# TimD1/vcfdist

Hardware: AMD Instinct MI355X
Metric: supercluster-alignments/sec (higher is better)
Workload: dtype int32; 1 GPU; wgs_synth; superclusters_per_gpu=1000000, span_dist=lognormal(median 20, sigma 1.2) clip [4,10000]

## Files before the change

### vcfdist_amd/csrc/pr_api.hip

```cpp
#include <hip/hip_runtime.h>
#include <hip/hip_ext.h>
#include <dlfcn.h>

#include <algorithm>
#include <atomic>
#include <chrono>
#include <cstdarg>
#include <cstdio>
#include <cstdlib>
#include <cstring>
#include <condition_variable>
#include <deque>
#include <functional>
#include <mutex>
#include <string>
#include <thread>
#include <tuple>
#include <unordered_map>
#include <unordered_set>
#include <vector>

#include "../../include/vcfdist_pr.h"
#include "pr_device.h"
#include "pr_plan.h"
// ... 910 lines not shown
    {
        static const int tie_model = vpr_selfcheck_tie_model(14);
        if (tie_model < 0)
            return fail(nullptr, VPR_ERR_STATE, "this machine's libstdc++ grows std::unordered_set through other bucket counts than the tie "
                        "replay's model (entry %d of TIE_BUCKET_LIST, pr_tie.hip): results on alignments with tied swap predecessors "
                        "would differ from a reference built here", -tie_model - 1);
    }
    int ndev = 0;
    hipError_t e = hipGetDeviceCount(&ndev);
    if (e != hipSuccess || ndev <= 0)
        return fail(nullptr, VPR_ERR_DEVICE, "no HIP device available (%s); this library has no CPU fallback",
                    e == hipSuccess ? "device count 0" : hipGetErrorString(e));
    if (cfg->device < 0 || cfg->device >= ndev)
        return fail(nullptr, VPR_ERR_ARG, "device %d out of range (have %d)", cfg->device, ndev);
    vpr_handle *h = new vpr_handle();
    h->cfg = *cfg;
    h->debug = getenv("VPR_DEBUG") != nullptr;
    h->no_strips = getenv("VPR_NO_STRIPS") != nullptr;
    h->no_round_overlap = getenv("VPR_NO_ROUND_OVERLAP") != nullptr;
    h->stall_log = getenv("VPR_STALL_LOG") != nullptr;
    h->seq_walk = getenv("VPR_SEQ_WALK") != nullptr;
    h->no_flag_save = getenv("VPR_NO_FLAG_SAVE") != nullptr;
    h->side_credit = exp_getenv("VPR_NO_SIDE_CREDIT") == nullptr;
    if (const char *e = exp_getenv("VPR_ZL_LDS_KB")) h->zl_lds_bytes = std::max(0, std::min(64, atoi(e))) * 1024;
    if (const char *e = exp_getenv("VPR_LANE_PRIO_ROWS")) h->lane_prio_rows = std::max(1, atoi(e));
    for (int k = 0; k < 2; k++)
        if (hipEventCreateWithFlags(&h->ev_cred[k], hipEventDisableTiming) != hipSuccess) return fail(nullptr, VPR_ERR_DEVICE, "hipEventCreate failed");
    if (const char *e = getenv("VPR_LONG_LT")) { const int v = atoi(e); if (v >= 64 && v <= 2048) h->long_lt = v; }
    memset(&h->dB, 0, sizeof(h->dB));
    memset(&h->timing, 0, sizeof(h->timing));
    const char *prio_map = exp_getenv("VPR_STREAM_PRIO");
    if (prio_map && strlen(prio_map) != size_t(N_CLASSES + 5)) prio_map = nullptr;
    if (hipSetDevice(cfg->device) != hipSuccess) { delete h; return fail(nullptr, VPR_ERR_DEVICE, "hipSetDevice failed"); }
    int prio_lo = 0, prio_hi = 0;
    (void)hipDeviceGetStreamPriorityRange(&prio_lo, &prio_hi);
    auto prio_of = [&](int idx, int dflt) { return !prio_map ? dflt : (prio_map[idx] == 'h' ? prio_hi : (prio_map[idx] == 'l' ? prio_lo : (prio_hi + prio_lo) / 2)); };
    if (hipStreamCreateWithPriority(&h->stream, exp_getenv("VPR_MAIN_BLOCKING") ? hipStreamDefault : hipStreamNonBlocking, prio_of(N_CLASSES + 4, (prio_hi + prio_lo) / 2)) != hipSuccess) {
        delete h;
        return fail(nullptr, VPR_ERR_DEVICE, "hipStreamCreate failed");
    }
    {
        size_t free_b = 0, total_b = 0;
        if (hipMemGetInfo(&free_b, &total_b) != hipSuccess) { delete h; return fail(nullptr, VPR_ERR_DEVICE, "hipMemGetInfo failed"); }
        h->dev_total = int64_t(total_b);
        h->tie_scratch_max = std::max<int64_t>(h->dev_total / 16, int64_t(64) << 20);
        h->lad_arena_max = std::max<int64_t>(h->dev_total / 8, int64_t(64) << 20);
// ... 1226 lines not shown
        });
        if (rc) return rc;
        }
        if (!(phases & 4)) return rc;
        const bool wave_walk = !q16 && (long_part || cnt < 2048);
        int64_t walk_rows_sum = 0;
        if (lv == LV_C1 && !h->seq_walk)
            for (int32_t k = 0; k < cnt && walk_rows_sum <= WSEG_MAX_ROWS; k++) walk_rows_sum += plan_desc(h, P, size_t(off) + size_t(k)).Lt;
        const bool seg_walk = lv == LV_C1 && !h->seq_walk && walk_rows_sum <= WSEG_MAX_ROWS;
        const bool row_walk = lv == LV_C1 && (wave_walk || seg_walk);
        vpr_launch_stat ws_;
        memset(&ws_, 0, sizeof(ws_));
        ws_.threads = q16 ? 16 : 64; ws_.n_units = cnt; ws_.cells_per_thread = 2;
        if (q16) {
            if (!zero) rc = timed(3, ws_, ks, "k_walk_q16", [&] {
                hipLaunchKernelGGL(k_walk_q16, dim3((cnt + 3) / 4), dim3(64), 0, ks, h->dB, h->d_descs, list, cnt,
                                   P.arena, a_i32, h->d_outs, a_path, tag, dtag, n_dev);
            });
            if (rc) return rc;
            ws_.cells_per_thread = 3;
            if (zero) {
                ws_.bytes_algorithmic = 20 * zl_rows;
                rc = timed(3, ws_, ks, "k_zero_walk", [&] {
                    hipLaunchKernelGGL(k_zero_walk, dim3((cnt + 63) / 64), dim3(64), 0, ks, h->d_descs, list, cnt, h->d_zl_hdr + zl_wave0,
                                       h->d_zl_in, h->d_zl_log, h->d_outs, a_path, (h->cfg.flags & VPR_CFG_KEEP_PATHS) ? 1 : 0, tag,
                                       h->lane_prio_rows);
                });
                if (rc) return rc;
                ws_.bytes_algorithmic = 0;
            }
            if (zero) rc = timed(3, ws_, ks, "k_zero_credit", [&] {
                hipLaunchKernelGGL(k_zero_credit, dim3((cnt + 63) / 64), dim3(64), 0, ks, h->dB, h->d_descs, list, cnt,
                                   h->d_zl_hdr + zl_wave0, h->d_zl_log, h->d_outs, h->d_secs, h->d_fp_table, h->d_jobs,
                                   h->d_njobs, h->jobs_cap, tag);
            });
            else if (cnt <= CREDIT_WAVE_MAX && !n_dev) rc = timed(3, ws_, ks, "k_credit<wave>", [&] {
                hipLaunchKernelGGL(k_credit<true>, dim3(cnt), dim3(64), 0, ks, h->dB, h->d_descs, list, cnt,
                                   h->d_outs, a_path, h->d_secs, h->d_fp_table, h->d_jobs, h->d_njobs,
                                   h->jobs_cap, dtag, tag, n_dev);
            });
            else {
                static const int head_max = [] { const char *e = exp_getenv("VPR_CREDIT_HEAD"); return e ? atoi(e) : 4096; }();
                const int32_t head = (n_dev && h->d_d1_blk && cnt > 2 * head_max) ? head_max : 0;
                if (head > 0) {
                    vpr_launch_stat wh_ = ws_;
                    wh_.n_units = head;
                    rc = timed(3, wh_, ks, "k_credit<wave>", [&] {
                        hipLaunchKernelGGL(k_credit<true>, dim3(head), dim3(64), 0, ks, h->dB, h->d_descs, list, head,
                                           h->d_outs, a_path, h->d_secs, h->d_fp_table, h->d_jobs, h->d_njobs,
                                           h->jobs_cap, dtag, tag, n_dev, 0);
                    });
                    if (rc) return rc;
                }
                rc = timed(3, ws_, ks, "k_credit<lane>", [&] {
                    hipLaunchKernelGGL(k_credit<false>, dim3((cnt - head + 63) / 64), dim3(64), 0, ks, h->dB, h->d_descs,
// ... 77 lines not shown
        const int nw = (cap + 63) / 64;
        vpr_launch_stat ls;
        memset(&ls, 0, sizeof(ls));
        ls.threads = 64; ls.cells_per_thread = 1; ls.n_units = cap;
        int rc = VPR_OK;
        if (ph == 1) {
            rc = timed(0, ls, ks, "k_prep_d1", [&] {
                hipLaunchKernelGGL(k_d1_hdr, dim3(nw), dim3(64), 0, ks, h->d_descs, list, n_dev, cap, h->d_outs, h->d_d1_hdr);
                hipLaunchKernelGGL(k_d1_scan, dim3(1), dim3(D1_SCAN_NT), 0, ks, h->d_d1_hdr, nw, h->d1_in_cap, h->d1_log_cap, h->d_d1_info);
                hipLaunchKernelGGL(k_prep_d1, dim3(nw), dim3(256), 0, ks, h->dB, h->d_descs, list, n_dev, cap, h->d_outs, h->d_d1_hdr, h->d_d1_in);
            });
            if (rc) return rc;
            rc = timed(1, ls, ks, "k_one_lane", [&] {
                hipLaunchKernelGGL(k_one_lane, dim3(nw), dim3(64), 0, ks, h->d_descs, list, n_dev, cap, h->d_d1_hdr, h->d_d1_in, h->d_d1_log,
                                   h->d_outs, reinterpret_cast<PathEnt *>(h->plan0.arena), (h->cfg.flags & VPR_CFG_KEEP_PATHS) ? 1 : 0, h->d_d1_info,
                                   std::max(1, h->lane_prio_rows / 4));
                hipLaunchKernelGGL(k_fwd_band_finish, dim3((cap + 255) / 256), dim3(256), 0, ks, list, cap, h->d_outs, D1_TAG, n_dev);
            });
            if (rc) return rc;
            ordered_fails(list, n_all, h->d_d1_fail, h->d_d1_info + 2, n_dev, ks);
        } else if (ph == 4) {
            ls.cells_per_thread = 3;
            rc = timed(3, ls, ks, "k_one_walk", [&] {
                hipLaunchKernelGGL(k_one_walk, dim3(nw), dim3(64), 0, ks, h->d_descs, list, n_dev, cap, h->d_d1_hdr, h->d_d1_in, h->d_d1_log,
                                   h->d_outs, reinterpret_cast<PathEnt *>(h->plan0.arena), (h->cfg.flags & VPR_CFG_KEEP_PATHS) ? 1 : 0, h->d_d1_info,
                                   std::max(1, h->lane_prio_rows / 4));
            });
            if (rc) return rc;
            rc = timed(3, ls, ks, "k_one_credit", [&] {
                hipLaunchKernelGGL(k_one_credit, dim3(nw), dim3(64), 0, ks, h->dB, h->d_descs, list, n_dev, cap, h->d_d1_hdr, h->d_d1_log,
                                   h->d_outs, h->d_secs, h->d_fp_table, h->d_jobs, h->d_njobs, h->jobs_cap, ztag);
            });
        }
        return rc;
    }

    int read_fails(int slot, int64_t fail_off, hipStream_t ls, std::vector<int32_t> &fails) {
        HIPCHK(h, x_event_sync(h, h->ev_slot[slot], SITE));
        const int32_t nf = h->hp_cnt[slot];
        if (nf > 0) {
            const size_t f0 = fails.size();
            fails.insert(fails.end(), h->hp_fail + fail_off, h->hp_fail + fail_off + nf);
            if (h->debug && nf <= (getenv("VPR_DEBUG_REJECTS") ? atoi(getenv("VPR_DEBUG_REJECTS")) : 64)) {
                for (size_t k = f0; k < fails.size(); k++) {
                    const int32_t a = fails[k];
                    AlnOut o;
                    (void)hipMemcpyAsync(&o, h->d_outs + a, sizeof(o), hipMemcpyDeviceToHost, ls);
                    (void)x_sync(h, ls, SITE);
                    const AlnDesc &d = h->descs[a];
                    fprintf(stderr, "[vpr] level %d rejected sc %d aln %d: Lq %d Lr %d Lt %d  s %d exit_min %d dq %d dr %d\n",
                            int(h->level[a]), d.sc, d.aln, d.Lq, d.Lr, d.Lt, o.s, o.exit_min, o.dist_q, o.dist_r);
                }
            }
// ... 910 lines not shown
```

### vcfdist_amd/csrc/pr_d1.hip

```cpp
#ifndef PR_D1_HIP_
#define PR_D1_HIP_

#define D1_TAG 9
#define D1_CLEAN ZL_CLEAN_REJECT

#define GE_ALIVE 1u
#define GE_MAT 2u
#define GE_SWP 4u
#define GE_PSLOT_SHIFT 3
#define GE_SUB 32u
#define GE_SUB_SHIFT 6
#define GE_INS 256u
#define GE_INS_SHIFT 9
#define GE_DEL 2048u
#define GE_DEL_SHIFT 12
#define GE_TP 16384u
#define GE_BWD 32768u

#define MV_SWP_R 0
#define MV_MAT 1
#define MV_SUB 2
#define MV_INS 3
#define MV_DEL 4
#define MV_SWP_Q 5
// ... 582 lines not shown
        zl_u4 pg_n = g_row(bmax - 1);
        for (int t = bmax - 1; t >= 0; t--) {
            const bool act = t < nrow;
            const bool first = act && t == nrow - 1;
            const zl_u2 pf = pf_n;
            const zl_u4 pgv = pg_n;
            pf_n = f_row(t - 1);
            pg_n = g_row(t - 1);
            const bool upper = act && ((((cf[0] | cf[1] | pf.x | pf.y) & 0xffff0000u) | cg[0][1] | cg[1][1] | pgv.y | pgv.w) != 0u);
#ifdef D1_CLOCKS
            if (lane == 0) { atomicAdd(info + 14, 1); if (__any(upper)) atomicAdd(info + 15, 1); }
#endif
            if (__any(upper)) sc_row(S4{}, t, act, first, pf, pgv);
            else sc_row(S2{}, t, act, first, pf, pgv);
        }
        beg_plane = kf[0][0] >= 0 ? VPR_PLANE_QUERY : VPR_PLANE_REF;
        ok = ok && (kf[0][0] >= 0 || kf[1][0] >= 0);
    }

    lapck(2);
    if (ok) { AlnOut &o = outs[a]; o.beg_plane = beg_plane; o.path_len = -1; }
}

__global__ void __launch_bounds__(64, 8) k_one_walk(const AlnDesc *__restrict__ descs, const int32_t *__restrict__ list,
                                                    const int32_t *__restrict__ n_dev, int n_cap, const ZlWave *__restrict__ hdr,
                                                    const uint32_t *__restrict__ zin, uint4 *__restrict__ zlog,
                                                    AlnOut *__restrict__ outs, PathEnt *__restrict__ paths, int keep_paths,
                                                    int32_t *__restrict__ info, int prio_rows) {
    const int w = blockIdx.x, lane = threadIdx.x;
    const ZlWave H = hdr[w];
    if (H.mt <= 0) return;
    if (H.mt >= prio_rows) __builtin_amdgcn_s_setprio(2);
    const int n_list = min(*n_dev, n_cap);
    const int wi = w * 64 + lane;
    const int a_ = wi < n_list ? list[wi] : -1;
    const int a = max(a_, 0);
    const AlnDesc *dp = descs + a;
    const bool ok = a_ >= 0 && outs[a].band_ok == D1_TAG && outs[a].path_len == -1;
    const int Lq = ok ? dp->Lq : 1, Lr = ok ? dp->Lr : 1;
    const int L[2] = {Lq, Lr};
    const int nrow = ok ? dp->Lt : 0;
    int bmax = nrow;
#pragma unroll
    for (int o = 32; o; o >>= 1) bmax = max(bmax, __shfl_xor(bmax, o));
    if (bmax == 0) return;
    const auto rin = __builtin_amdgcn_make_buffer_rsrc(const_cast<uint32_t *>(zin + H.in_off), 0, 256 * (2 * H.mq + 2 * H.mr + H.mt), 0x00020000);
    const auto rlog = __builtin_amdgcn_make_buffer_rsrc(zlog + H.log_off, 0, 2560 * (H.mt + 1), 0x00020000);
    const uint32_t lane4 = uint32_t(lane) << 2, lane8 = uint32_t(lane) << 3, lane16 = uint32_t(lane) << 4;
    const uint32_t posW[2] = {0u, uint32_t(2 * H.mq) << 8};
    const uint32_t post = uint32_t(2 * H.mq + 2 * H.mr) << 8;
    const uint32_t logB1 = uint32_t(H.mt + 1) << 10;
    auto in_at = [&](uint32_t off) -> uint32_t { return __builtin_amdgcn_raw_buffer_load_b32(rin, off, 0, 0); };
    auto word_at = [&](int p, int x, bool on) -> uint32_t { return in_at(on ? posW[p] + (uint32_t(x) << 8) + lane4 : ZL_OOB); };
    auto t_at = [&](int t, bool on) -> uint32_t { return in_at(on ? post + (uint32_t(t) << 8) + lane4 : ZL_OOB); };
    const int beg_plane = ok ? outs[a].beg_plane : 0;
    auto lapck = [&](int) {};
    {
        PathEnt *path = paths + dp->path_off;
        const uint32_t logS0 = logB1;
        int hi = beg_plane, slot = 0, layer = 0, x = 0, ti = 0, mv_in = -1;
        uint32_t status = 0;
        bool wok = ok, done = !ok;
        int plen = 0;
        for (int i = 0; i <= bmax; i++) {
            const bool act = wok && !done;
            if (!__any(act)) break;
            const uint32_t mvw = __builtin_amdgcn_raw_buffer_load_b32(rlog, act ? (uint32_t(ti) << 10) + lane16 + (uint32_t(layer) << 3) + (uint32_t(hi) << 2) : ZL_OOB, 0, 0);
            const uint32_t tw = t_at(ti, act);
            const uint32_t cw = word_at(hi, x, act);
            const int trv = ZW_PTR(tw), qref = hi ? x : ZW_PTR(cw);
            uint32_t sync = 1, edit = 0;
            if (mv_in >= 0) {
                const bool diag = mv_in != MV_INS && mv_in != MV_DEL;
                const bool in_t = (tw & ZW_PV) && !(tw & ZW_PB);
                const bool in_q = hi == 0 && (cw & ZW_PV) && !(cw & ZW_PB);
                sync = (diag && !in_t && !in_q && !((tw | cw) & ZW_INS) && trv == qref) ? 1u : 0u;
                edit = (mv_in == MV_SUB || mv_in == MV_INS || mv_in == MV_DEL) ? 1u : 0u;
            }
            const uint32_t eqb = (ZW_BASE(cw) == ZW_BASE(tw) ? 1u : 0u) | ((hi || !(cw & ZW_PV)) ? 2u : 0u);
            zl_u2 st;
            st.x = uint32_t(x) | (uint32_t(hi) << 16) | (sync << 17) | (eqb << 18) | (edit << 20) | (uint32_t(i - ti) << 21);
            st.y = uint32_t(qref + 1) | (uint32_t(trv + 1) << 16);
            __builtin_amdgcn_raw_buffer_store_b64(st, rlog, act ? logS0 + (uint32_t(i) << 9) + lane8 : ZL_OOB, 0, 0);
            if ((keep_paths & 1) && act) {
                uint4 pe;
                pe.x = uint32_t(x) | (uint32_t(hi) << 31);
                pe.y = uint32_t(ti) | (sync << 31) | (edit << 30);
                pe.z = uint32_t(qref);
                pe.w = uint32_t(trv);
                *reinterpret_cast<uint4 *>(path + i) = pe;
            }
            if (act) {
                if (layer == 1 && hi == 0 && x == Lq - 1 && ti == nrow - 1) { done = true; plen = i + 1; }
                else {
                    const uint32_t m = (mvw >> (8 * slot)) & 0xffu;
                    const int rank = int(m & 7u), to = int((m >> 3) & 3u);
                    if (m == 0xffu) { status |= VPR_ST_ERR_NO_PTR; wok = false; }
                    else if (rank == MV_MAT) { x++; ti++; }
                    else if (rank == MV_SWP_R || rank == MV_SWP_Q) { x = ZW_PTR(cw) + 1; hi = 1 - hi; slot = to; ti++; }
                    else if (rank == MV_SUB) { x++; ti++; layer = 1; slot = to; }
                    else if (rank == MV_INS) { x++; layer = 1; slot = to; }
                    else { ti++; layer = 1; slot = to; }
                    mv_in = rank;
                    if (ti >= nrow || x >= L[hi]) { status |= VPR_ST_ERR_NO_PTR; wok = false; }
                }
            }
        }
        lapck(3);
        {
            const int nf = __popcll(__ballot(ok && wok && done));
            if (lane == 0 && nf) atomicAdd(info + 4, nf);
        }
        if (ok) {
            AlnOut &o = outs[a];
            wok = wok && done;
            if (!wok) status |= VPR_ST_ERR_NO_PTR;
            o.beg_plane = beg_plane;
            o.path_len = wok ? plen : 0;
            if (!wok) o.n_sec = 0;
            if (status) atomicOr(&o.status, status);
        }
    }
}

struct D1Fetch {
    const uint2 *log;
    int64_t pre_i;
    uint2 pre;
    __device__ PathEnt operator()(int64_t i) {
        const uint2 v = (i == pre_i) ? pre : log[i * 64];
        if (i > 0) { pre_i = i - 1; pre = log[(i - 1) * 64]; }
        PathEnt e;
        e.a = (v.x & 0xffffu) | (((v.x >> 16) & 1u) << 31);
        e.b = uint32_t(i - int64_t((v.x >> 21) & 1u)) | (((v.x >> 17) & 1u) << 31) | (((v.x >> 20) & 1u) << 30) | (((v.x >> 18) & 3u) << 28);
        e.qref = int(v.y & 0xffffu) - 1;
        e.tref = int(v.y >> 16) - 1;
        return e;
    }
};

__global__ void __launch_bounds__(64) k_one_credit(DevBatch B, const AlnDesc *__restrict__ descs, const int32_t *__restrict__ list,
                                                   const int32_t *__restrict__ n_dev, int n_cap, const ZlWave *__restrict__ hdr,
                                                   const uint4 *__restrict__ zlog, AlnOut *__restrict__ outs, Section *__restrict__ secs,
                                                   int32_t *const *__restrict__ fp_group, EdJob *__restrict__ jobs,
                                                   int32_t *__restrict__ n_jobs, int32_t jobs_cap, int ztag) {
    const int w = blockIdx.x, lane = threadIdx.x;
    const ZlWave H = hdr[w];
    if (H.mt <= 0) return;
    const int wi = w * 64 + lane;
    if (wi >= min(*n_dev, n_cap)) return;
    const int a = list[wi];
    if (a < 0) return;
    const AlnDesc d = descs[a];
    AlnOut &O = outs[a];
    if (d.band_pad != ztag || O.band_ok != D1_TAG) return;
    if (O.status & (VPR_ST_ERR_NO_PTR | VPR_ST_ERR_LIMIT)) return;
    D1Fetch f{reinterpret_cast<const uint2 *>(zlog + H.log_off + 64 * (int64_t(H.mt) + 1)) + lane, -1, make_uint2(0, 0)};
    credit_walk<false, D1Fetch, true>(B, d, O, a, nullptr, int64_t(O.path_len), 0u, secs, fp_group, jobs, n_jobs, jobs_cap, true, f);
}

#endif
```

### vcfdist_amd/csrc/pr_host.h

```cpp
#ifndef PR_HOST_H_
#define PR_HOST_H_
#include <hip/hip_runtime.h>
#include <hip/hip_ext.h>

#include <algorithm>
#include <atomic>
#include <chrono>
#include <cstdarg>
#include <cstdio>
#include <cstdlib>
#include <cstring>
#include <condition_variable>
#include <deque>
#include <functional>
#include <mutex>
#include <string>
#include <thread>
#include <tuple>
#include <unordered_map>
#include <unordered_set>
#include <vector>

#include "../../include/vcfdist_pr.h"
#include "pr_device.h"
// ... 264 lines not shown
    int32_t *d_fail = nullptr, *d_cnt = nullptr;
    int4 *d_tie_list = nullptr, *hp_tie_list = nullptr; int32_t tie_list_cap = 0;
    int32_t *hp_flag = nullptr; int32_t flag_seq = 0;
    int32_t *d_tie_cnt = nullptr, *hp_tie_cnt = nullptr;
    hipEvent_t ev_spec = nullptr;
    TieJob *hp_tie_jobs = nullptr; size_t tie_jobs_cap = 0;
    int4 *d_tie_dec = nullptr; int64_t tie_dec_cap = 0;
    int32_t *d_tie_ndec = nullptr;
    std::vector<int32_t> plan0_pos;
    ZlWave *d_zl_hdr = nullptr; uint32_t *d_zl_in = nullptr; uint4 *d_zl_log = nullptr;
    std::vector<int64_t> zl_wave0;
    ZlWave *d_d1_hdr = nullptr; uint32_t *d_d1_in = nullptr; uint4 *d_d1_log = nullptr; int32_t *d_d1_fail = nullptr, *d_d1_info = nullptr;
    int32_t *d_d1_blk = nullptr;
    hipEvent_t ev_offsets = nullptr;
    hipEvent_t ev_cred[2] = {nullptr, nullptr};
    bool side_credit = true;
    struct Plan0Pass {
        bool valid = false, bad = false;
        int64_t part_cells[2] = {0, 0}, part_in[2] = {0, 0}, part_dense[2] = {0, 0}, part_rows[2] = {0, 0}, need128 = 0, need_max = 0;
        std::vector<std::pair<int64_t, int32_t>> big;
    } p0;
    int64_t d1_in_cap = 0, d1_log_cap = 0;
    int32_t d1_wave_cap = 0, d1_fail_cap = 0;
    int32_t d1_max_rows = 256;
    std::vector<ZlWave> zl_hdr_host;
    int32_t long_lt = LONG_LT;
    const vpr_variants *gen_src = nullptr;
    uint8_t *d_ctg_seq = nullptr; const uint8_t *ctg_src = nullptr; int64_t ctg_bytes = 0; uint64_t ctg_probe = 0;
    int32_t *hp_fail = nullptr, *hp_cnt = nullptr;
    std::vector<void *> pinned;
    int32_t *d_ed_scratch = nullptr; size_t ed_scratch_ints = 0;
    int64_t ed_max_len = -1;
    std::vector<EvPair> events;
    std::vector<hipEvent_t> ev_pool; size_t ev_used = 0;
    std::vector<hipStream_t> pad_streams;
    int zl_lds_bytes = 0;
    int lane_prio_rows = 256;
    DevResults dR;
    DistState *dist = nullptr;
    vpr_timing timing;
    bool uploaded = false, executed = false;
};

int fail(vpr_handle *h, int code, const char *fmt, ...);
const char *vpr_create_error();
#define HIPCHK(h, call)                                                                         \
// ... 47 lines not shown
```

### vcfdist_amd/csrc/pr_kernels.hip

```cpp
#include <hip/hip_runtime.h>
#include <stdint.h>

#include "../../include/vcfdist_pr.h"
#include "pr_device.h"
#include "pr_scan.h"

__device__ __forceinline__ bool fwd_allow(int f) { return !(f & PV) || (f & PE); }
__device__ __forceinline__ bool bwd_allow(int f) { return !(f & PV) || (f & PB); }

__global__ void __launch_bounds__(256) k_prep_scof(DevBatch B) {
    __shared__ int64_t s_off[257];
    const int which = blockIdx.y;
    const int64_t *off = which < 4 ? B.hap_off[which] : B.ref_off;
    int32_t *out = which < 4 ? B.sc_hap[which] : B.sc_ref;
    const int sc0 = blockIdx.x * 256, m = min(256, B.n_sc - sc0);
    for (int i = threadIdx.x; i <= m; i += 256) s_off[i] = off[sc0 + i];
    __syncthreads();
    const int64_t beg = s_off[0], end = s_off[m];
    for (int64_t g = beg + threadIdx.x; g < end; g += 256) {
        int lo = 0, hi = m;
        while (hi - lo > 1) {
            const int mid = (lo + hi) >> 1;
            if (s_off[mid] <= g) lo = mid; else hi = mid;
        }
// ... 517 lines not shown
    if (tie_used) { atomicOr(&outs[a].status, VPR_ST_SWAP_TIE); outs[a].band_ok = TIE_MARK(0); atomicAdd(&outs[a].n_sec, int(tie_used)); }
}

#undef FROW

#define ED_INLINE_LONG 256
__device__ int small_ed(const uint8_t *a, int m, const uint8_t *b, int n) {
    int row[33];
    for (int j = 0; j <= n; j++) row[j] = j;
    for (int i = 1; i <= m; i++) {
        int diag = row[0];
        row[0] = i;
        const uint8_t ai = a[i - 1];
        for (int j = 1; j <= n; j++) {
            const int up = row[j];
            const int v = min(min(up + 1, row[j - 1] + 1), diag + (ai != b[j - 1]));
            diag = up;
            row[j] = v;
        }
    }
    return row[n];
}

struct NoFetch { __device__ PathEnt operator()(int64_t) const { return PathEnt{0, 0, 0, 0}; } };
template <bool WAVE, class XF = NoFetch, bool EXT = false>
__device__ __forceinline__ void credit_walk(const DevBatch &B, const AlnDesc &d, AlnOut &O, const int a,
                                            const PathEnt *__restrict__ path, const int64_t n, uint32_t status,
                                            Section *__restrict__ secs, int32_t *const *__restrict__ fp_group,
                                            EdJob *__restrict__ jobs, int32_t *__restrict__ n_jobs, int32_t jobs_cap,
                                            const bool lead, XF xf = XF()) {
    const int qi = 0, ri = 1;
    const int32_t *q2r = B.hap_ptr[d.qs] + d.q_off;
    const int32_t *t2r = B.hap_ptr[d.ts] + d.t_off;
    const int q_size = d.Lq, r_size = d.Lr, t_size = d.Lt;
    (void)qi;
    const uint8_t *Rs = B.ref_seq + d.r_off;
    const uint8_t *Ts = B.hap_seq[d.ts] + d.t_off;
    const int swap = (d.aln == 1 || d.aln == 2);
    const int32_t *qv_pos = B.var_pos[d.qs];
    const int32_t *tv_pos = B.var_pos[d.ts];
    int32_t *fpg = fp_group[d.qs * 2 + swap];
    Section *sec = secs + d.sec_off;
    int n_sec = 0;

    int sync_group = 0;
    const int end_hi = O.end_plane;
    int cur_hi = end_hi;
// ... 84 lines not shown
                ts_base = max(0, i - 63);
                const int x = ts_base + lane_;
                ts_cur = x < t_size ? int(Ts[x]) : 0;
            }
            return __builtin_amdgcn_readlane(ts_cur, i - ts_base);
        } else {
            return int(Ts[i]);
        }
    };

    bool clean = false;
    int64_t pl_base = -1;
    bool pl_static = false;
    auto plain_static = [&]() {
        const int qr = ccur.qref, ti = int(ccur.b & 0x0fffffffu);
        const bool have = cbase + lane_ < n;
        const bool eqb = have && qr >= 0 && qr < r_size && ti < t_size && Rs[qr] == Ts[ti];
        const int qr_up = __shfl_down(qr, 1), ti_up = __shfl_down(ti, 1);
        const bool eq_up = __shfl_down(int(eqb), 1) != 0;
        pl_static = have && lane_ < 63 && cbase + lane_ + 1 < n && (ccur.b >> 31) && !((ccur.b >> 30) & 1u) &&
                    qr_up == qr + 1 && ti_up == ti + 1 && eq_up;
        pl_base = cbase;
    };
    while (sync_idx >= 0) {
        if constexpr (WAVE && !EXT) {
            if (clean && sync_idx < n) {
                if (pl_base != cbase) plain_static();
                const int l = int(sync_idx - cbase);
                const bool plain = pl_static && ccur.qref >= query_var_pos && ccur.tref >= truth_var_pos;
                const unsigned long long below = (l == 63) ? ~0ull : ((2ull << l) - 1ull);
                const unsigned long long stop = ~__ballot(plain) & below;
                const int run = stop ? l - (63 - __builtin_clzll(stop)) : l + 1;
                if (run > 0) {
                    const int lj = l - run + 1;
                    prev_qref = __builtin_amdgcn_readlane(ccur.qref, lj);
                    prev_tref = __builtin_amdgcn_readlane(ccur.tref, lj);
                    cur_b = uint32_t(__builtin_amdgcn_readlane(int(ccur.b), lj));
                    prev_hi = int(uint32_t(__builtin_amdgcn_readlane(int(ccur.a), lj)) >> 31);
                    prev_ti = int(cur_b & 0x0fffffffu);
                    prev_sync_ref_idx = prev_qref + 1;
                    prev_sync_truth_idx = prev_ti + 1;
                    eq_cur = (cur_b >> 28) & 3u;
                    sync_idx -= run;
                    if (sync_idx < 0) break;
                    cur_hi = prev_hi;
                    const PathEnt e = fetch(sync_idx);
// ... 63 lines not shown
            const int sync_ref_idx = prev_qref + 1;
            const int sync_truth_idx = prev_ti + 1;
            int rl = prev_sync_ref_idx - sync_ref_idx, tl = prev_sync_truth_idx - sync_truth_idx;
            if (rl < 0 || rl > r_size - sync_ref_idx) rl = r_size - sync_ref_idx;
            if (tl < 0 || tl > t_size - sync_truth_idx) tl = t_size - sync_truth_idx;
            const bool has_q = query_var_ptr != prev_query_var_ptr;
            const bool has_t = truth_var_ptr != prev_truth_var_ptr;
            int ref_ed = -1;
            bool deferred = false;
            if (rl == 0) ref_ed = tl;
            else if (tl == 0) ref_ed = rl;
            else if (rl == 1 && tl == 1)
                ref_ed = ((eq_next & 2u) && nx_qref == sync_ref_idx && nx_ti == sync_truth_idx) ? int(!(eq_next & 1u))
                                                                                                : int(rs_at(sync_ref_idx) != ts_at(sync_truth_idx));
            else if (!has_q && !has_t && rl == tl) {
                bool same = true;
                for (int k = rl - 1; k >= 0 && same; k--) same = (rs_at(sync_ref_idx + k) == ts_at(sync_truth_idx + k));
                if (same) ref_ed = 0;
            }
            if (ref_ed < 0) {
                if (tl <= 32 && rl <= ED_INLINE_LONG) ref_ed = small_ed(Rs + sync_ref_idx, rl, Ts + sync_truth_idx, tl);
                else if (rl <= 32 && tl <= ED_INLINE_LONG) ref_ed = small_ed(Ts + sync_truth_idx, tl, Rs + sync_ref_idx, rl);
                else deferred = true;
            }
            if (has_q || has_t || deferred) {
                if (n_sec < d.sec_cap) {
                    Section S;
                    S.q_lo = int32_t(query_var_ptr); S.q_hi = int32_t(prev_query_var_ptr);
                    S.t_lo = int32_t(truth_var_ptr); S.t_hi = int32_t(prev_truth_var_ptr);
                    S.sync_group = sync_group; S.query_ed = query_ed; S.ref_ed = ref_ed;
                    S.flags = (deferred ? SEC_DEFERRED : 0) | ((has_q || has_t) ? 0 : SEC_NOVAR);
                    if (deferred && lead) {
                        const int32_t j = atomicAdd(n_jobs, 1);
                        if (j < jobs_cap) jobs[j] = EdJob{a, n_sec, sync_ref_idx, rl, sync_truth_idx, tl};
                        else status |= VPR_ST_ERR_LIMIT;
                    }
                    if (lead) sec[n_sec] = S;
                    n_sec++;
                } else status |= VPR_ST_ERR_LIMIT;
            } else {
                if (ref_ed != 0) status |= VPR_ST_WARN_REF_ED;
                if (query_ed != ref_ed) status |= VPR_ST_WARN_QUERY_ED;
                if (query_ed > ref_ed) status |= VPR_ST_WARN_EXCEEDS;
            }
            if (has_q || has_t) sync_group++;
            prev_query_var_ptr = query_var_ptr;
// ... 612 lines not shown
```

### vcfdist_amd/csrc/pr_zl.hip

```cpp
#ifndef PR_ZL_HIP_
#define PR_ZL_HIP_
#include <type_traits>


#define ZW_PTR(w) (int((w) & 0xffffu) - 1)
#define ZW_BASE(w) (((w) >> 16) & 0x7fu)
#define ZW_PV (1u << 23)
#define ZW_PB (1u << 24)
#define ZW_PE (1u << 25)
#define ZW_INS (1u << 26)
#define ZW_TP (1u << 27)
__device__ __forceinline__ bool zw_fwd_allow(uint32_t w) { return !(w & ZW_PV) || (w & ZW_PE); }
__device__ __forceinline__ bool zw_bwd_allow(uint32_t w) { return !(w & ZW_PV) || (w & ZW_PB); }

#define ZE_ALIVE 1u
#define ZE_HASMAT 2u
#define ZE_HASSWP 4u
#define ZE_PSLOT_SHIFT 3
#define ZE_TP 32u
#define ZE_BWD 64u

#define ZL_MAXLEN 65000
#define ZL_CLEAN_REJECT (-1)

// ... 314 lines not shown
            for (int p = 0; p < 2; p++) {
#pragma unroll
                for (int s = 0; s < 4; s++) sc[p][s] = (p == ep && s == es) ? 0 : -1;
            }
        }
        next_reg = row_at(t - 4);
        const zl_u2 pre = pre_reg;
        const bool upper = act && (((cur.x | cur.y | pre.x | pre.y) & 0xffff0000u) != 0u);
        if (__any(upper)) bwd_row(std::integral_constant<int, 4>{}, t, act, pre);
        else bwd_row(std::integral_constant<int, 2>{}, t, act, pre);
        lastpre = pre;
    };
    for (int t = bmax - 1; t >= 1; t -= 4) {
        bwd_step(t, rA, rD);
        bwd_step(t - 1, rB, rA);
        bwd_step(t - 2, rC, rB);
        bwd_step(t - 3, rD, rC);
    }
    const int beg_plane = sc[0][0] >= 0 ? VPR_PLANE_QUERY : VPR_PLANE_REF;

    if (ok) outs[a].beg_plane = beg_plane;
}

__global__ void __launch_bounds__(64, 8) k_zero_walk(const AlnDesc *__restrict__ descs, const int32_t *__restrict__ list, int n_list,
                                                  const ZlWave *__restrict__ hdr, const uint32_t *__restrict__ zin,
                                                  uint4 *__restrict__ zlog, AlnOut *__restrict__ outs, PathEnt *__restrict__ paths,
                                                  int keep_paths, int tag, int prio_rows) {
    const int w = blockIdx.x, lane = threadIdx.x;
    const ZlWave H = hdr[w];
    if (H.mt >= prio_rows) __builtin_amdgcn_s_setprio(2);
    const int wi = w * 64 + lane;
    const int a_ = wi < n_list ? list[wi] : -1;
    const bool live = a_ >= 0;
    const int a = max(a_, 0);
    const AlnDesc *dp = descs + a;
    const auto rin = __builtin_amdgcn_make_buffer_rsrc(const_cast<uint32_t *>(zin + H.in_off), 0, 256 * (H.mq + H.mr + H.mt), 0x00020000);
    const auto rlog = __builtin_amdgcn_make_buffer_rsrc(zlog + H.log_off, 0, 1280 * H.mt, 0x00020000);
    const uint32_t lane4 = uint32_t(lane) << 2, lane8 = uint32_t(lane) << 3;
    const uint32_t pos0[2] = {0u, uint32_t(H.mq) << 8}, post = uint32_t(H.mq + H.mr) << 8;
    const uint32_t logP0 = uint32_t(H.mt) << 9, logS0 = logP0 + (uint32_t(H.mt) << 8);
    auto in_at = [&](uint32_t off) -> uint32_t { return __builtin_amdgcn_raw_buffer_load_b32(rin, off, 0, 0); };
    const bool ok = live && dp->band_pad == tag && outs[a].band_ok == tag;
    const int nrow = ok ? dp->Lt : 0;
    int bmax = nrow;
#pragma unroll
    for (int o = 32; o; o >>= 1) bmax = max(bmax, __shfl_xor(bmax, o));
    if (bmax == 0) return;
    const int beg_plane = ok ? outs[a].beg_plane : 0;
    PathEnt *path = paths + dp->path_off;
    int hi = beg_plane, slot = 0, mv_in = 0, x = 0;
    uint32_t status = 0;
    bool wok = ok;
    for (int t = 0; t < bmax; t++) {
        const bool act = wok && t < nrow;
        const uint32_t ppw = __builtin_amdgcn_raw_buffer_load_b32(rlog, (act && t + 1 < nrow) ? logP0 + (uint32_t(t) << 8) + lane4 : ZL_OOB, 0, 0);
        const uint32_t tw = in_at(act ? post + (uint32_t(t) << 8) + lane4 : ZL_OOB);
        const uint32_t cw = in_at(act ? pos0[hi] + (uint32_t(x) << 8) + lane4 : ZL_OOB);
        const int trv = ZW_PTR(tw), qref = hi ? x : ZW_PTR(cw);
        uint32_t sync = 1;
        if (mv_in) {
            const bool in_t = (tw & ZW_PV) && !(tw & ZW_PB);
            const bool in_q = hi == 0 && (cw & ZW_PV) && !(cw & ZW_PB);
            sync = (!in_t && !in_q && !((tw | cw) & ZW_INS) && trv == qref) ? 1u : 0u;
        }
        const uint32_t eqb = (ZW_BASE(cw) == ZW_BASE(tw) ? 1u : 0u) | ((hi || !(cw & ZW_PV)) ? 2u : 0u);
        zl_u2 st;
        st.x = uint32_t(x) | (uint32_t(hi) << 16) | (sync << 17) | (eqb << 18);
        st.y = uint32_t(qref + 1) | (uint32_t(trv + 1) << 16);
        __builtin_amdgcn_raw_buffer_store_b64(st, rlog, act ? logS0 + (uint32_t(t) << 9) + lane8 : ZL_OOB, 0, 0);
        if ((keep_paths & 1) && act) {
            uint4 pe;
            pe.x = uint32_t(x) | (uint32_t(hi) << 31);
            pe.y = uint32_t(t) | (sync << 31);
            pe.z = uint32_t(qref);
            pe.w = uint32_t(trv);
            *reinterpret_cast<uint4 *>(path + t) = pe;
        }
        if (act && t + 1 < nrow) {
            const uint32_t nb = (ppw >> (4 * ((hi << 2) | slot))) & 15u;
            if (hi == 1 && (nb & 2u)) { hi = 0; slot = int(nb >> 2); x = ZW_PTR(cw) + 1; }
            else if (nb & 1u) { x = x + 1; }
            else if (hi == 0 && (nb & 2u)) { hi = 1; slot = int(nb >> 2); x = ZW_PTR(cw) + 1; }
            else { status |= VPR_ST_ERR_NO_PTR; wok = false; }
            mv_in = 1;
        }
    }
    if (ok) {
        AlnOut &o = outs[a];
        o.path_len = wok ? nrow : 0;
        if (!wok) o.n_sec = 0;
        if (status) atomicOr(&o.status, status);
    }
}

struct ZlFetch {
    const uint2 *log;
    int64_t pre_i;
    uint2 pre;
    __device__ PathEnt operator()(int64_t i) {
        const uint2 v = (i == pre_i) ? pre : log[i * 64];
        if (i > 0) { pre_i = i - 1; pre = log[(i - 1) * 64]; }
        PathEnt e;
        e.a = (v.x & 0xffffu) | (((v.x >> 16) & 1u) << 31);
        e.b = uint32_t(i) | (((v.x >> 17) & 1u) << 31) | (((v.x >> 18) & 3u) << 28);
        e.qref = int(v.y & 0xffffu) - 1;
        e.tref = int(v.y >> 16) - 1;
        return e;
    }
};

__global__ void __launch_bounds__(64) k_zero_credit(DevBatch B, const AlnDesc *__restrict__ descs, const int32_t *__restrict__ list,
                                                    int n_list, const ZlWave *__restrict__ hdr, const uint4 *__restrict__ zlog,
                                                    AlnOut *__restrict__ outs, Section *__restrict__ secs,
                                                    int32_t *const *__restrict__ fp_group, EdJob *__restrict__ jobs,
                                                    int32_t *__restrict__ n_jobs, int32_t jobs_cap, int tag) {
    const int w = blockIdx.x, lane = threadIdx.x;
    const int wi = w * 64 + lane;
    if (wi >= n_list) return;
    const int a = list[wi];
    if (a < 0) return;
    const AlnDesc d = descs[a];
    AlnOut &O = outs[a];
    if (d.band_pad != tag || O.band_ok != tag) return;
    if (O.status & (VPR_ST_ERR_NO_PTR | VPR_ST_ERR_LIMIT)) return;
    const ZlWave H = hdr[w];
    ZlFetch f{reinterpret_cast<const uint2 *>(zlog + H.log_off + 48 * int64_t(H.mt)) + lane, -1, make_uint2(0, 0)};
    credit_walk<false, ZlFetch, true>(B, d, O, a, nullptr, int64_t(O.path_len), 0u, secs, fp_group, jobs, n_jobs, jobs_cap, true, f);
}

#endif
```

Before: 194.6 million supercluster-alignments/s.

## Prefetch traceback rows ahead in lane walks and add optional LDS credit ring

The zero-lane and one-lane walk kernels now run in blocks of four rows. The predictable loads (pointer words and truth words) are fetched one block ahead, and the query words are fetched speculatively along the straight-line path, so each serial traceback step no longer waits on a dependent global load. This is on by default and can be disabled with an environment variable. A second path stages credit-walk log records through a per-lane LDS ring filled by buffer loads in batches of eight; it is off by default. The cost is higher register pressure, wasted loads when the path turns, and more code complexity.

```diff
diff --git a/vcfdist_amd/csrc/pr_api.hip b/vcfdist_amd/csrc/pr_api.hip
--- a/vcfdist_amd/csrc/pr_api.hip
+++ b/vcfdist_amd/csrc/pr_api.hip
@@ -956,6 +956,8 @@
     h->seq_walk = getenv("VPR_SEQ_WALK") != nullptr;
     h->no_flag_save = getenv("VPR_NO_FLAG_SAVE") != nullptr;
     h->side_credit = exp_getenv("VPR_NO_SIDE_CREDIT") == nullptr;
+    h->lane_ahead = getenv("VPR_LANE_ONE_AHEAD") == nullptr;
+    h->credit_ring = getenv("VPR_LANE_CREDIT_RING") != nullptr;
     if (const char *e = exp_getenv("VPR_ZL_LDS_KB")) h->zl_lds_bytes = std::max(0, std::min(64, atoi(e))) * 1024;
     if (const char *e = exp_getenv("VPR_LANE_PRIO_ROWS")) h->lane_prio_rows = std::max(1, atoi(e));
     for (int k = 0; k < 2; k++)
@@ -2228,7 +2230,7 @@
             if (zero) {
                 ws_.bytes_algorithmic = 20 * zl_rows;
                 rc = timed(3, ws_, ks, "k_zero_walk", [&] {
-                    hipLaunchKernelGGL(k_zero_walk, dim3((cnt + 63) / 64), dim3(64), 0, ks, h->d_descs, list, cnt, h->d_zl_hdr + zl_wave0,
+                    hipLaunchKernelGGL((h->lane_ahead ? k_zero_walk<true> : k_zero_walk<false>), dim3((cnt + 63) / 64), dim3(64), 0, ks, h->d_descs, list, cnt, h->d_zl_hdr + zl_wave0,
                                        h->d_zl_in, h->d_zl_log, h->d_outs, a_path, (h->cfg.flags & VPR_CFG_KEEP_PATHS) ? 1 : 0, tag,
                                        h->lane_prio_rows);
                 });
@@ -2236,7 +2238,7 @@
                 ws_.bytes_algorithmic = 0;
             }
             if (zero) rc = timed(3, ws_, ks, "k_zero_credit", [&] {
-                hipLaunchKernelGGL(k_zero_credit, dim3((cnt + 63) / 64), dim3(64), 0, ks, h->dB, h->d_descs, list, cnt,
+                hipLaunchKernelGGL((h->credit_ring ? k_zero_credit<true> : k_zero_credit<false>), dim3((cnt + 63) / 64), dim3(64), 0, ks, h->dB, h->d_descs, list, cnt,
                                    h->d_zl_hdr + zl_wave0, h->d_zl_log, h->d_outs, h->d_secs, h->d_fp_table, h->d_jobs,
                                    h->d_njobs, h->jobs_cap, tag);
             });
@@ -2360,13 +2362,13 @@
         } else if (ph == 4) {
             ls.cells_per_thread = 3;
             rc = timed(3, ls, ks, "k_one_walk", [&] {
-                hipLaunchKernelGGL(k_one_walk, dim3(nw), dim3(64), 0, ks, h->d_descs, list, n_dev, cap, h->d_d1_hdr, h->d_d1_in, h->d_d1_log,
+                hipLaunchKernelGGL((h->lane_ahead ? k_one_walk<true> : k_one_walk<false>), dim3(nw), dim3(64), 0, ks, h->d_descs, list, n_dev, cap, h->d_d1_hdr, h->d_d1_in, h->d_d1_log,
                                    h->d_outs, reinterpret_cast<PathEnt *>(h->plan0.arena), (h->cfg.flags & VPR_CFG_KEEP_PATHS) ? 1 : 0, h->d_d1_info,
                                    std::max(1, h->lane_prio_rows / 4));
             });
             if (rc) return rc;
             rc = timed(3, ls, ks, "k_one_credit", [&] {
-                hipLaunchKernelGGL(k_one_credit, dim3(nw), dim3(64), 0, ks, h->dB, h->d_descs, list, n_dev, cap, h->d_d1_hdr, h->d_d1_log,
+                hipLaunchKernelGGL((h->credit_ring ? k_one_credit<true> : k_one_credit<false>), dim3(nw), dim3(64), 0, ks, h->dB, h->d_descs, list, n_dev, cap, h->d_d1_hdr, h->d_d1_log,
                                    h->d_outs, h->d_secs, h->d_fp_table, h->d_jobs, h->d_njobs, h->jobs_cap, ztag);
             });
         }
diff --git a/vcfdist_amd/csrc/pr_d1.hip b/vcfdist_amd/csrc/pr_d1.hip
--- a/vcfdist_amd/csrc/pr_d1.hip
+++ b/vcfdist_amd/csrc/pr_d1.hip
@@ -628,6 +628,7 @@
     if (ok) { AlnOut &o = outs[a]; o.beg_plane = beg_plane; o.path_len = -1; }
 }
 
+template <bool AHEAD>
 __global__ void __launch_bounds__(64, 8) k_one_walk(const AlnDesc *__restrict__ descs, const int32_t *__restrict__ list,
                                                     const int32_t *__restrict__ n_dev, int n_cap, const ZlWave *__restrict__ hdr,
                                                     const uint32_t *__restrict__ zin, uint4 *__restrict__ zlog,
@@ -668,12 +669,7 @@
         uint32_t status = 0;
         bool wok = ok, done = !ok;
         int plen = 0;
-        for (int i = 0; i <= bmax; i++) {
-            const bool act = wok && !done;
-            if (!__any(act)) break;
-            const uint32_t mvw = __builtin_amdgcn_raw_buffer_load_b32(rlog, act ? (uint32_t(ti) << 10) + lane16 + (uint32_t(layer) << 3) + (uint32_t(hi) << 2) : ZL_OOB, 0, 0);
-            const uint32_t tw = t_at(ti, act);
-            const uint32_t cw = word_at(hi, x, act);
+        auto walk_step = [&](const int i, const bool act, const uint32_t mvw, const uint32_t tw, const uint32_t cw) {
             const int trv = ZW_PTR(tw), qref = hi ? x : ZW_PTR(cw);
             uint32_t sync = 1, edit = 0;
             if (mv_in >= 0) {
@@ -711,6 +707,59 @@
                     if (ti >= nrow || x >= L[hi]) { status |= VPR_ST_ERR_NO_PTR; wok = false; }
                 }
             }
+        };
+        auto mv_at = [&](int t, int ly, int p, bool on) -> uint32_t {
+            return __builtin_amdgcn_raw_buffer_load_b32(rlog, on ? (uint32_t(t) << 10) + lane16 + (uint32_t(ly) << 3) + (uint32_t(p) << 2) : ZL_OOB, 0, 0);
+        };
+        if constexpr (!AHEAD) {
+            for (int i = 0; i <= bmax; i++) {
+                const bool act = wok && !done;
+                if (!__any(act)) break;
+                const uint32_t mvw = mv_at(ti, layer, hi, act);
+                const uint32_t tw = t_at(ti, act);
+                const uint32_t cw = word_at(hi, x, act);
+                walk_step(i, act, mvw, tw, cw);
+            }
+        } else {
+            constexpr int R = WALK_AHEAD;
+            for (int i0 = 0; i0 <= bmax; i0 += R) {
+                if (!__any(wok && !done)) break;
+                uint32_t mv[R], tq[R], sw[R];
+#pragma unroll
+                for (int j = 0; j < R; j++) { mv[j] = 0; tq[j] = 0; sw[j] = 0; }
+                int s_t0 = 0, s_x0 = 0, s_lp = -1, s_end = 0;
+                auto scout = [&](auto Jc, const bool want) {
+                    constexpr int J = decltype(Jc)::value;
+                    bool on[R];
+                    uint32_t mvv[R], twv[R], cwv[R];
+                    int end = J;
+#pragma unroll
+                    for (int k = J; k < R; k++) {
+                        const int d = k - J;
+                        on[k] = want && (d == 0 || (i0 + k <= bmax && ti + d < nrow && x + d < L[hi]));
+                        mvv[k] = mv_at(ti + d, layer, hi, on[k]);
+                        twv[k] = t_at(ti + d, on[k]);
+                        cwv[k] = word_at(hi, x + d, on[k]);
+                        end = on[k] ? k + 1 : end;
+                    }
+#pragma unroll
+                    for (int k = J; k < R; k++) { mv[k] = on[k] ? mvv[k] : mv[k]; tq[k] = on[k] ? twv[k] : tq[k]; sw[k] = on[k] ? cwv[k] : sw[k]; }
+                    s_t0 = want ? ti - J : s_t0; s_x0 = want ? x - J : s_x0; s_lp = want ? layer * 2 + hi : s_lp; s_end = want ? end : s_end;
+                };
+                auto step = [&](auto Jc) {
+                    constexpr int J = decltype(Jc)::value;
+                    const int i = i0 + J;
+                    const bool act = wok && !done && i <= bmax;
+                    const bool need = act && !(J < s_end && ti == s_t0 + J && x == s_x0 + J && layer * 2 + hi == s_lp);
+                    if (__any(need)) scout(Jc, need);
+                    walk_step(i, act, act ? mv[J] : 0u, act ? tq[J] : 0u, act ? sw[J] : 0u);
+                };
+                static_assert(R == 4, "the block below names its steps");
+                step(std::integral_constant<int, 0>{});
+                step(std::integral_constant<int, 1>{});
+                step(std::integral_constant<int, 2>{});
+                step(std::integral_constant<int, 3>{});
+            }
         }
         lapck(3);
         {
@@ -743,8 +792,21 @@
         e.tref = int(v.y >> 16) - 1;
         return e;
     }
+    __device__ void settle() const {}
 };
 
+struct D1Step {
+    __device__ __forceinline__ PathEnt operator()(uint2 v, int64_t i) const {
+        PathEnt e;
+        e.a = (v.x & 0xffffu) | (((v.x >> 16) & 1u) << 31);
+        e.b = uint32_t(i - int64_t((v.x >> 21) & 1u)) | (((v.x >> 17) & 1u) << 31) | (((v.x >> 20) & 1u) << 30) | (((v.x >> 18) & 3u) << 28);
+        e.qref = int(v.y & 0xffffu) - 1;
+        e.tref = int(v.y >> 16) - 1;
+        return e;
+    }
+};
+
+template <bool RING>
 __global__ void __launch_bounds__(64) k_one_credit(DevBatch B, const AlnDesc *__restrict__ descs, const int32_t *__restrict__ list,
                                                    const int32_t *__restrict__ n_dev, int n_cap, const ZlWave *__restrict__ hdr,
                                                    const uint4 *__restrict__ zlog, AlnOut *__restrict__ outs, Section *__restrict__ secs,
@@ -761,8 +823,16 @@
     AlnOut &O = outs[a];
     if (d.band_pad != ztag || O.band_ok != D1_TAG) return;
     if (O.status & (VPR_ST_ERR_NO_PTR | VPR_ST_ERR_LIMIT)) return;
-    D1Fetch f{reinterpret_cast<const uint2 *>(zlog + H.log_off + 64 * (int64_t(H.mt) + 1)) + lane, -1, make_uint2(0, 0)};
-    credit_walk<false, D1Fetch, true>(B, d, O, a, nullptr, int64_t(O.path_len), 0u, secs, fp_group, jobs, n_jobs, jobs_cap, true, f);
+    const uint4 *steps = zlog + H.log_off + 64 * (int64_t(H.mt) + 1);
+    if constexpr (RING) {
+        __shared__ uint2 ring[LANE_RING][64];
+        const int n = O.path_len;
+        RingFetch<D1Step> f(__builtin_amdgcn_make_buffer_rsrc(const_cast<uint4 *>(steps), 0, 512 * (H.mt + 1), 0x00020000), ring, n);
+        credit_walk<false, RingFetch<D1Step>, true>(B, d, O, a, nullptr, int64_t(n), 0u, secs, fp_group, jobs, n_jobs, jobs_cap, true, f);
+    } else {
+        D1Fetch f{reinterpret_cast<const uint2 *>(steps) + lane, -1, make_uint2(0, 0)};
+        credit_walk<false, D1Fetch, true>(B, d, O, a, nullptr, int64_t(O.path_len), 0u, secs, fp_group, jobs, n_jobs, jobs_cap, true, f);
+    }
 }
 
 #endif
diff --git a/vcfdist_amd/csrc/pr_host.h b/vcfdist_amd/csrc/pr_host.h
--- a/vcfdist_amd/csrc/pr_host.h
+++ b/vcfdist_amd/csrc/pr_host.h
@@ -310,6 +310,8 @@
     } p0;
     int64_t d1_in_cap = 0, d1_log_cap = 0;
     int32_t d1_wave_cap = 0, d1_fail_cap = 0;
+    bool lane_ahead = true;
+    bool credit_ring = false;
     int32_t d1_max_rows = 256;
     std::vector<ZlWave> zl_hdr_host;
     int32_t long_lt = LONG_LT;
diff --git a/vcfdist_amd/csrc/pr_kernels.hip b/vcfdist_amd/csrc/pr_kernels.hip
--- a/vcfdist_amd/csrc/pr_kernels.hip
+++ b/vcfdist_amd/csrc/pr_kernels.hip
@@ -563,7 +563,7 @@
     return row[n];
 }
 
-struct NoFetch { __device__ PathEnt operator()(int64_t) const { return PathEnt{0, 0, 0, 0}; } };
+struct NoFetch { __device__ PathEnt operator()(int64_t) const { return PathEnt{0, 0, 0, 0}; } __device__ void settle() const {} };
 template <bool WAVE, class XF = NoFetch, bool EXT = false>
 __device__ __forceinline__ void credit_walk(const DevBatch &B, const AlnDesc &d, AlnOut &O, const int a,
                                             const PathEnt *__restrict__ path, const int64_t n, uint32_t status,
@@ -694,6 +694,7 @@
                     qr_up == qr + 1 && ti_up == ti + 1 && eq_up;
         pl_base = cbase;
     };
+    if constexpr (EXT) xf.settle();
     while (sync_idx >= 0) {
         if constexpr (WAVE && !EXT) {
             if (clean && sync_idx < n) {
@@ -803,6 +804,7 @@
                 if (tl <= 32 && rl <= ED_INLINE_LONG) ref_ed = small_ed(Rs + sync_ref_idx, rl, Ts + sync_truth_idx, tl);
                 else if (rl <= 32 && tl <= ED_INLINE_LONG) ref_ed = small_ed(Ts + sync_truth_idx, tl, Rs + sync_ref_idx, rl);
                 else deferred = true;
+                if constexpr (EXT) xf.settle();
             }
             if (has_q || has_t || deferred) {
                 if (n_sec < d.sec_cap) {
diff --git a/vcfdist_amd/csrc/pr_zl.hip b/vcfdist_amd/csrc/pr_zl.hip
--- a/vcfdist_amd/csrc/pr_zl.hip
+++ b/vcfdist_amd/csrc/pr_zl.hip
@@ -360,6 +360,8 @@
     if (ok) outs[a].beg_plane = beg_plane;
 }
 
+#define WALK_AHEAD 4
+template <bool AHEAD>
 __global__ void __launch_bounds__(64, 8) k_zero_walk(const AlnDesc *__restrict__ descs, const int32_t *__restrict__ list, int n_list,
                                                   const ZlWave *__restrict__ hdr, const uint32_t *__restrict__ zin,
                                                   uint4 *__restrict__ zlog, AlnOut *__restrict__ outs, PathEnt *__restrict__ paths,
@@ -389,11 +391,7 @@
     int hi = beg_plane, slot = 0, mv_in = 0, x = 0;
     uint32_t status = 0;
     bool wok = ok;
-    for (int t = 0; t < bmax; t++) {
-        const bool act = wok && t < nrow;
-        const uint32_t ppw = __builtin_amdgcn_raw_buffer_load_b32(rlog, (act && t + 1 < nrow) ? logP0 + (uint32_t(t) << 8) + lane4 : ZL_OOB, 0, 0);
-        const uint32_t tw = in_at(act ? post + (uint32_t(t) << 8) + lane4 : ZL_OOB);
-        const uint32_t cw = in_at(act ? pos0[hi] + (uint32_t(x) << 8) + lane4 : ZL_OOB);
+    auto walk_row = [&](const int t, const bool act, const uint32_t ppw, const uint32_t tw, const uint32_t cw) {
         const int trv = ZW_PTR(tw), qref = hi ? x : ZW_PTR(cw);
         uint32_t sync = 1;
         if (mv_in) {
@@ -421,6 +419,66 @@
             else if (hi == 0 && (nb & 2u)) { hi = 1; slot = int(nb >> 2); x = ZW_PTR(cw) + 1; }
             else { status |= VPR_ST_ERR_NO_PTR; wok = false; }
             mv_in = 1;
+        }
+    };
+    if constexpr (!AHEAD) {
+        for (int t = 0; t < bmax; t++) {
+            const bool act = wok && t < nrow;
+            const uint32_t ppw = __builtin_amdgcn_raw_buffer_load_b32(rlog, (act && t + 1 < nrow) ? logP0 + (uint32_t(t) << 8) + lane4 : ZL_OOB, 0, 0);
+            const uint32_t tw = in_at(act ? post + (uint32_t(t) << 8) + lane4 : ZL_OOB);
+            const uint32_t cw = in_at(act ? pos0[hi] + (uint32_t(x) << 8) + lane4 : ZL_OOB);
+            walk_row(t, act, ppw, tw, cw);
+        }
+    } else {
+        constexpr int R = WALK_AHEAD;
+        auto pp_at = [&](int t) -> uint32_t {
+            return __builtin_amdgcn_raw_buffer_load_b32(rlog, (ok && t + 1 < nrow) ? logP0 + (uint32_t(t) << 8) + lane4 : ZL_OOB, 0, 0);
+        };
+        auto tw_at = [&](int t) -> uint32_t { return in_at((ok && t < nrow) ? post + (uint32_t(t) << 8) + lane4 : ZL_OOB); };
+        auto stays = [](uint32_t ppw, int hi_, int slot_) -> bool {
+            const uint32_t nb = (ppw >> (4 * ((hi_ << 2) | slot_))) & 15u;
+            return !(hi_ == 1 && (nb & 2u)) && (nb & 1u);
+        };
+        uint32_t np[R], nt[R];
+#pragma unroll
+        for (int j = 0; j < R; j++) { np[j] = pp_at(j); nt[j] = tw_at(j); }
+        for (int t0 = 0; t0 < bmax; t0 += R) {
+            uint32_t cp[R], ct[R], sw[R];
+#pragma unroll
+            for (int j = 0; j < R; j++) { cp[j] = np[j]; ct[j] = nt[j]; sw[j] = 0; }
+#pragma unroll
+            for (int j = 0; j < R; j++) { np[j] = pp_at(t0 + R + j); nt[j] = tw_at(t0 + R + j); }
+            int s_hi = 0, s_x0 = 0, s_end = 0;
+            auto scout = [&](auto Jc, const bool want) {
+                constexpr int J = decltype(Jc)::value;
+                bool run = want, on[R];
+                uint32_t wv[R];
+                int end = J;
+#pragma unroll
+                for (int k = J; k < R; k++) {
+                    run = run && t0 + k < nrow;
+                    on[k] = run;
+                    wv[k] = in_at(run ? pos0[hi] + (uint32_t(x + k - J) << 8) + lane4 : ZL_OOB);
+                    end = run ? k + 1 : end;
+                    run = run && stays(cp[k], hi, slot);
+                }
+#pragma unroll
+                for (int k = J; k < R; k++) sw[k] = on[k] ? wv[k] : sw[k];
+                s_hi = want ? hi : s_hi; s_x0 = want ? x - J : s_x0; s_end = want ? end : s_end;
+            };
+            auto row = [&](auto Jc) {
+                constexpr int J = decltype(Jc)::value;
+                const int t = t0 + J;
+                const bool act = wok && t < nrow;
+                const bool need = act && !(J < s_end && hi == s_hi && x == s_x0 + J);
+                if (__any(need)) scout(Jc, need);
+                walk_row(t, act, cp[J], ct[J], act ? sw[J] : 0u);
+            };
+            static_assert(R == 4, "the block below names its rows");
+            row(std::integral_constant<int, 0>{});
+            row(std::integral_constant<int, 1>{});
+            row(std::integral_constant<int, 2>{});
+            row(std::integral_constant<int, 3>{});
         }
     }
     if (ok) {
@@ -445,14 +503,66 @@
         e.tref = int(v.y >> 16) - 1;
         return e;
     }
+    __device__ void settle() const {}
 };
 
+#define LANE_RING 8
+typedef decltype(__builtin_amdgcn_make_buffer_rsrc(static_cast<void *>(nullptr), short(0), 0, 0)) zl_rsrc;
+typedef uint2 (*zl_ring)[64];
+template <class DEC>
+struct RingFetch {
+    zl_rsrc rs;
+    zl_ring ring;
+    int k;
+    int next_i;
+    zl_u2 nx[LANE_RING];
+    __device__ __forceinline__ zl_u2 rec(int i) const {
+        return __builtin_amdgcn_raw_buffer_load_b64(rs, i >= 0 ? (uint32_t(i) << 9) + (uint32_t(threadIdx.x) << 3) : ZL_OOB, 0, 0);
+    }
+    __device__ __forceinline__ RingFetch(zl_rsrc rs_, zl_ring ring_, int n) : rs(rs_), ring(ring_), k(0), next_i(n - 1) {
+#pragma unroll
+        for (int j = 0; j < LANE_RING; j++) nx[j] = rec(next_i - j);
+    }
+    __device__ __forceinline__ PathEnt operator()(int64_t i) {
+        int r = k & (LANE_RING - 1);
+        const bool other = int64_t(r == 0 ? next_i : next_i + LANE_RING - r) != i;
+        if (r == 0 || other) {
+            if (other) {
+                next_i = int(i);
+                k = r = 0;
+#pragma unroll
+                for (int j = 0; j < LANE_RING; j++) nx[j] = rec(next_i - j);
+            }
+#pragma unroll
+            for (int j = 0; j < LANE_RING; j++) ring[j][threadIdx.x] = make_uint2(nx[j].x, nx[j].y);
+            next_i -= LANE_RING;
+#pragma unroll
+            for (int j = 0; j < LANE_RING; j++) nx[j] = rec(next_i - j);
+        }
+        k++;
+        return DEC()(ring[r][threadIdx.x], i);
+    }
+    __device__ __forceinline__ void settle() const { __builtin_amdgcn_s_waitcnt(0x0f70); }
+};
+struct ZlStep {
+    __device__ __forceinline__ PathEnt operator()(uint2 v, int64_t i) const {
+        PathEnt e;
+        e.a = (v.x & 0xffffu) | (((v.x >> 16) & 1u) << 31);
+        e.b = uint32_t(i) | (((v.x >> 17) & 1u) << 31) | (((v.x >> 18) & 3u) << 28);
+        e.qref = int(v.y & 0xffffu) - 1;
+        e.tref = int(v.y >> 16) - 1;
+        return e;
+    }
+};
+
+template <bool RING>
 __global__ void __launch_bounds__(64) k_zero_credit(DevBatch B, const AlnDesc *__restrict__ descs, const int32_t *__restrict__ list,
                                                     int n_list, const ZlWave *__restrict__ hdr, const uint4 *__restrict__ zlog,
                                                     AlnOut *__restrict__ outs, Section *__restrict__ secs,
                                                     int32_t *const *__restrict__ fp_group, EdJob *__restrict__ jobs,
                                                     int32_t *__restrict__ n_jobs, int32_t jobs_cap, int tag) {
     const int w = blockIdx.x, lane = threadIdx.x;
+    const ZlWave H = hdr[w];
     const int wi = w * 64 + lane;
     if (wi >= n_list) return;
     const int a = list[wi];
@@ -461,9 +571,16 @@
     AlnOut &O = outs[a];
     if (d.band_pad != tag || O.band_ok != tag) return;
     if (O.status & (VPR_ST_ERR_NO_PTR | VPR_ST_ERR_LIMIT)) return;
-    const ZlWave H = hdr[w];
-    ZlFetch f{reinterpret_cast<const uint2 *>(zlog + H.log_off + 48 * int64_t(H.mt)) + lane, -1, make_uint2(0, 0)};
-    credit_walk<false, ZlFetch, true>(B, d, O, a, nullptr, int64_t(O.path_len), 0u, secs, fp_group, jobs, n_jobs, jobs_cap, true, f);
+    const uint4 *steps = zlog + H.log_off + 48 * int64_t(H.mt);
+    if constexpr (RING) {
+        __shared__ uint2 ring[LANE_RING][64];
+        const int n = O.path_len;
+        RingFetch<ZlStep> f(__builtin_amdgcn_make_buffer_rsrc(const_cast<uint4 *>(steps), 0, 512 * H.mt, 0x00020000), ring, n);
+        credit_walk<false, RingFetch<ZlStep>, true>(B, d, O, a, nullptr, int64_t(n), 0u, secs, fp_group, jobs, n_jobs, jobs_cap, true, f);
+    } else {
+        ZlFetch f{reinterpret_cast<const uint2 *>(steps) + lane, -1, make_uint2(0, 0)};
+        credit_walk<false, ZlFetch, true>(B, d, O, a, nullptr, int64_t(O.path_len), 0u, secs, fp_group, jobs, n_jobs, jobs_cap, true, f);
+    }
 }
 
 #endif
```

Result: no change. 193.6 million supercluster-alignments/s (median of 2 runs) (-0.5%).
